# CPJKU/audio_sheet_retrieval

Hardware: AMD Instinct MI355X
Metric: snippet-pairs/sec embedded+ranked (32-d CCA) (higher is better)
Workload: dtype f32

## Files before the change

audio_sheet_retrieval_amd/csrc/conv_wino_kernels.hip:

```cpp
#include <hip/hip_runtime.h>
#include <stdint.h>
#include <stdlib.h>
#include <algorithm>
#include <vector>
#include "asr_kernels.h"
#include "repack_elems.inl"
#include "wino_tile_order.h"

#ifndef ASR_WINOG_ABL
#define ASR_WINOG_ABL 0
#endif

namespace asr {

typedef float floatx4w __attribute__((ext_vector_type(4)));
typedef float float2w __attribute__((ext_vector_type(2)));

#ifndef ASR_WINO_ASMREAD
#define ASR_WINO_ASMREAD 1
#endif
#ifndef ASR_WINO_BUFDMA
#define ASR_WINO_BUFDMA 1
#endif

struct WinoArgs {
    const float *in;
    const float *wpk;
    const float *bnp;
    float *out;
    int N, H, W, OH, OW;
    int RY, RX;
    int MY, MX;
    int nmy, nmx;
    int tiles_y, tiles_x;
    int coutp;
    int C4P, RP;
    int total;
    int per;
    double *stats;
    BnBwdFuse bf;
    const void *raw;
    const float *w1;
    const float *bn1;
};

#ifndef ASR_WINO_PKADD
#define ASR_WINO_PKADD 1
#endif
__device__ __forceinline__ float ssub(float a, float b) {
    float r;
    asm("v_sub_f32 %0, %1, %2" : "=v"(r) : "v"(a), "v"(b));
    return r;
}
__device__ __forceinline__ float2w psub(float2w a, float2w b) {
    if (ASR_WINO_PKADD) return a - b;
    return float2w{ssub(a[0], b[0]), ssub(a[1], b[1])};
}
__device__ __forceinline__ floatx4w psub(floatx4w a, floatx4w b) {
    if (ASR_WINO_PKADD) return a - b;
    return floatx4w{ssub(a[0], b[0]), ssub(a[1], b[1]), ssub(a[2], b[2]), ssub(a[3], b[3])};
}
__device__ __forceinline__ float sadd(float a, float b) {
    float r;
    asm("v_add_f32 %0, %1, %2" : "=v"(r) : "v"(a), "v"(b));
    return r;
}
// ... 7 lines not shown
}

__device__ float4 g_wino_zero[4];

template <int NTV>
__device__ __forceinline__ void wino_stats_store(double *stats, int row, int cout, int col0, int lane,
                                                 const double (&s1)[NTV], const double (&s2)[NTV]) {
    const int g = lane >> 4, n = lane & 15;
#pragma unroll
    for (int nt = 0; nt < NTV; ++nt) {
        double a = s1[nt], b = s2[nt];
        a += __shfl_xor(a, 16); b += __shfl_xor(b, 16);
        a += __shfl_xor(a, 32); b += __shfl_xor(b, 32);
        const int ch = col0 + nt * 16 + n;
        if (g == 0 && ch < cout) {
            stats[((size_t)row * 2) * cout + ch] = a;
            stats[((size_t)row * 2 + 1) * cout + ch] = b;
        }
    }
}

__device__ __forceinline__ float elu_fastw(float y) { return y > 0.0f ? y : __expf(y) - 1.0f; }

template <int CIN, int COUT, bool POOL, int NTW, int KB, int WAVES, int MINW, int RMAX, bool RAW, int PW = 0,
          int IN_MODE = 0>
__global__ __launch_bounds__(64 * (WAVES + PW), MINW) void conv3x3_wino(WinoArgs a) {
    constexpr int KS = CIN / 4;
    constexpr int NB = CIN / 8;
    constexpr bool REM = (CIN % 8) != 0;
    constexpr int NCH = NB / KB;
    constexpr int WROW = NTW * 16;
    constexpr int WS = NTW == 2 ? 48 : WROW;
    constexpr int C4 = CIN / 4;
    constexpr int T = 64 * (WAVES + PW);
    static_assert(NB % KB == 0, "chunking must divide the channel blocks");
    static_assert(PW == 0 || (!RAW && NTW * 16 >= COUT), "producer builds: deterministic path, one n-group");
    extern __shared__ __align__(16) float lds[];
    const int tid = threadIdx.x, lane = tid & 63;
    const int wave = __builtin_amdgcn_readfirstlane(tid >> 6);
    const int LW = a.RX + 2, LH = a.RY + 2;
    constexpr int C4P = (C4 & 1) ? C4 : C4 + 1;
    constexpr int CSf = C4P * 4;
    const int RPf = a.RP * 4;
    const int buf_floats = (LH * RPf + 255) & ~255;
    float *w_lds = lds + 2 * buf_floats;
    const int ng = blockIdx.y;
    const int first = blockIdx.x * a.per;
    const int last = min(first + a.per, a.total);
    if (first >= last) return;

    for (int i = tid; i < 16 * KS * 4 * (WROW / 4); i += T) {
        const int row = i / (WROW / 4), q = i - row * (WROW / 4);
        const int col = ng * WROW + q * 4;
        float4 v = make_float4(0.f, 0.f, 0.f, 0.f);
        if (col < a.coutp) v = *reinterpret_cast<const float4 *>(a.wpk + (size_t)row * a.coutp + col);
        *reinterpret_cast<float4 *>(w_lds + row * WS + q * 4) = v;
    }
    constexpr int RMAXE = PW > 0 ? 1 : RMAX;
    int st_g[RMAXE], st_rc[RMAXE];
    if constexpr (PW == 0) {
#pragma unroll
        for (int k = 0; k < RMAX; ++k) {
            const int f = tid + k * T;
            const int r = f / a.RP;
            const int xs = f - r * a.RP - ((r >> 1) & 1);
            const int px = xs / C4P, c = xs - px * C4P;
            const bool real = r < LH && xs >= 0 && px < LW && c < C4;
#if ASR_WINO_BUFDMA
            st_g[k] = real ? (((r - 1) * a.W + (px - 1)) * CIN + c * 4) * 4 : (int)0x80000000;
#else
            st_g[k] = ((r - 1) * a.W + (px - 1)) * CIN + c * 4;
#endif
            st_rc[k] = real ? (r << 16) | px : -1;
        }
    }
    auto fetch = [&](int region, float *buf) {
        if constexpr (PW == 0) {
        const int tx = region % a.tiles_x;
        const int rest = region / a.tiles_x;
        const int ty = rest % a.tiles_y;
        const int img = rest / a.tiles_y;
        const int Y0 = ty * a.RY, X0 = tx * a.RX;
#if ASR_WINO_BUFDMA
        {
            typedef int int4v __attribute__((ext_vector_type(4)));
            const uint64_t ibase = reinterpret_cast<uint64_t>(a.in + (int64_t)img * a.H * a.W * CIN);
            int4v rsrc;
            rsrc.x = (int)(uint32_t)ibase;
            rsrc.y = (int)(uint32_t)(ibase >> 32);
            rsrc.z = a.H * a.W * CIN * 4;
            rsrc.w = 0x00020000;
            const int roff = (Y0 * a.W + X0) * CIN * 4;
            const unsigned lds0 = (unsigned)(uintptr_t)(__attribute__((address_space(3))) void *)buf;
            const bool xedge = X0 < 1 || X0 + LW - 1 > a.W;
            auto dma = [&](int k, int vo) {
                const unsigned m0v = lds0 + (unsigned)((k * T + wave * 64) * 16);
                asm volatile("s_mov_b32 m0, %2\n\ts_nop 0\n\tbuffer_load_dwordx4 %0, %1, 0 offen lds"
                             ::"v"(vo), "s"(rsrc), "s"(m0v)
                             : "memory", "m0");
            };
            if (!__builtin_amdgcn_readfirstlane((int)xedge)) {
#pragma unroll
                for (int k = 0; k < RMAX; ++k) {
                    if ((k * T + wave * 64) * 4 >= buf_floats) break;
// ... 74 lines not shown
#pragma unroll 1
            for (int cg = 0; cg < C4; ++cg) {
                const float *wg = a.w1 + cg * 36;
                float res[4];
#pragma unroll
                for (int c = 0; c < 4; ++c) {
                    const int co = cg * 4 + c;
                    float acc = 0.0f;
#pragma unroll
                    for (int t = 0; t < 9; ++t) acc = fmaf(v[t], wg[c * 9 + t], acc);
                    res[c] = elu_fastw((acc - a.bn1[co]) * a.bn1[C1P + co] + a.bn1[2 * C1P + co]);
                }
                *reinterpret_cast<float4 *>(dst + cg * 4) = make_float4(res[0], res[1], res[2], res[3]);
            }
        }
        }
    };
    const bool producer = PW > 0 && wave >= WAVES;
    if constexpr (PW > 0) {
        if (IN_MODE == 2)
            for (int i = tid; i < 256; i += T) tab255[i] = (float)i / 255.0f;
        __syncthreads();
        if (producer) produce(first, lds);
    } else {
        fetch(first, lds);
#if ASR_WINO_BUFDMA
        asm volatile("s_waitcnt vmcnt(0)" ::: "memory");
#endif
    }
    __syncthreads();

    const int m = lane & 15, g = lane >> 4, n = lane & 15;
    const int tyy = m / a.MX, txx = m - tyy * a.MX;
    int a_row[4];
#pragma unroll
    for (int i = 0; i < 4; ++i)
        a_row[i] = (2 * tyy + i) * RPf + 2 * txx * CSf + ((tyy + (i >> 1)) & 1) * 4;
    const int a_pair = (g >> 1) * 4 + (g & 1) * 2;
    const int a_rem = NB * 8 + g;
    const float *w_lane = w_lds + g * WS + n;
    auto wq_off = [](int q) { return ((q / (16 * NTW)) * 16 + (q / NTW) % 16) * 4 * WS + (q % NTW) * 16; };
    int ey[4], ex[4], eoff[4];
#pragma unroll
    for (int r = 0; r < 4; ++r) {
        const int me = 4 * g + r;
        ey[r] = me / a.MX;
        ex[r] = me - ey[r] * a.MX;
        eoff[r] = (POOL ? ey[r] * a.OW + ex[r] : 2 * ey[r] * a.W + 2 * ex[r]) * COUT + ng * WROW + n;
    }
    float bmean[NTW], bscale[NTW], bbeta[NTW];
#pragma unroll
    for (int nt = 0; nt < NTW; ++nt) {
        const int ch = ng * WROW + nt * 16 + n;
        const bool ok = !RAW && ch < COUT;
        bmean[nt] = ok ? a.bnp[ch] : 0.f;
        bscale[nt] = ok ? a.bnp[a.coutp + ch] : 1.f;
        bbeta[nt] = ok ? a.bnp[2 * a.coutp + ch] : 0.f;
    }
    float bistd[NTW];
    const bool bnb = ASR_BNB_FUSE_BUILD && RAW && a.stats && a.bf.z != nullptr;
#pragma unroll
    for (int nt = 0; nt < NTW; ++nt) {
        const int ch = ng * WROW + nt * 16 + n;
        bistd[nt] = 0.f;
        if (bnb && ch < COUT) {
            bmean[nt] = a.bf.cst[ch]; bistd[nt] = a.bf.cst[COUT + ch];
            bscale[nt] = a.bf.cst[2 * COUT + ch]; bbeta[nt] = a.bf.cst[3 * COUT + ch];
        }
    }

    double st1[NTW], st2[NTW];
#pragma unroll
    for (int nt = 0; nt < NTW; ++nt) { st1[nt] = 0.0; st2[nt] = 0.0; }
    for (int region = first; region < last; ++region) {
    const float *in_lds = lds + ((region - first) & 1) * buf_floats;
    if (region + 1 < last && !(ASR_WINOG_ABL & 1)) {
        if constexpr (PW > 0) {
            if (producer) produce(region + 1, lds + ((region + 1 - first) & 1) * buf_floats);
        } else {
            fetch(region + 1, lds + ((region + 1 - first) & 1) * buf_floats);
        }
    }
    const int tx = region % a.tiles_x;
    const int rest = region / a.tiles_x;
    const int ty = rest % a.tiles_y;
    const int img = rest / a.tiles_y;
    const int Y0 = ty * a.RY, X0 = tx * a.RX;
    for (int mt = producer ? a.nmy * a.nmx : wave; mt < a.nmy * a.nmx; mt += WAVES) {
        const int mty = mt / a.nmx, mtx = mt - mty * a.nmx;
        const int oy = mty * a.MY * 2, ox = mtx * a.MX * 2;
        if (Y0 + oy >= a.H || X0 + ox >= a.W) continue;
        const float *ap = in_lds + oy * RPf + ox * CSf;
        floatx4w acc[16][NTW];
#pragma unroll
        for (int p = 0; p < 16; ++p)
#pragma unroll
            for (int nt = 0; nt < NTW; ++nt) acc[p][nt] = floatx4w{0.f, 0.f, 0.f, 0.f};

#pragma unroll
        for (int ch = 0; ch < NCH + (REM ? 1 : 0); ++ch) {
            if (ch < NCH) {
                float2w dp[4][4][KB];
#if ASR_WINO_ASMREAD
                if (ASR_WINOG_ABL & 32) {
#pragma unroll
                    for (int i = 0; i < 4; ++i)
#pragma unroll
                        for (int j = 0; j < 4; ++j)
#pragma unroll
                            for (int c = 0; c < KB; ++c) dp[i][j][c] = float2w{(float)i, (float)j};
                } else {
#pragma unroll
                    for (int i = 0; i < 4; ++i) {
                        const unsigned la = (unsigned)(uintptr_t)(const __attribute__((address_space(3))) void *)(ap + a_row[i] + a_pair);
#pragma unroll
                        for (int j = 0; j < 4; ++j)
#pragma unroll
                            for (int c = 0; c < KB; ++c)
                                asm volatile("ds_read_b64 %0, %1 offset:%2"
                                             : "=v"(dp[i][j][c])
                                             : "v"(la), "n"((j * CSf + (ch * KB + c) * 8) * 4));
                    }
#pragma unroll
                    for (int c = 0; c < KB; ++c)
                        asm volatile("s_waitcnt lgkmcnt(0)"
                                     : "+v"(dp[0][0][c]), "+v"(dp[0][1][c]), "+v"(dp[0][2][c]), "+v"(dp[0][3][c]),
                                       "+v"(dp[1][0][c]), "+v"(dp[1][1][c]), "+v"(dp[1][2][c]), "+v"(dp[1][3][c]),
                                       "+v"(dp[2][0][c]), "+v"(dp[2][1][c]), "+v"(dp[2][2][c]), "+v"(dp[2][3][c]),
                                       "+v"(dp[3][0][c]), "+v"(dp[3][1][c]), "+v"(dp[3][2][c]), "+v"(dp[3][3][c]));
                }
#else
#pragma unroll
                for (int i = 0; i < 4; ++i)
#pragma unroll
                    for (int j = 0; j < 4; ++j)
#pragma unroll
                        for (int c = 0; c < KB; ++c)
                            dp[i][j][c] = (ASR_WINOG_ABL & 32) ? float2w{(float)i, (float)j}
                                                               : *reinterpret_cast<const float2w *>(ap + a_row[i] + j * CSf + (ch * KB + c) * 8 + a_pair);
#endif
#pragma unroll
                for (int c = 0; c < KB; ++c) {
#pragma unroll
                    for (int j = 0; j < 4; ++j) {
                        const float2w d0 = dp[0][j][c], d1 = dp[1][j][c], d2 = dp[2][j][c], d3 = dp[3][j][c];
                        dp[0][j][c] = psub(d0, d2); dp[1][j][c] = padd(d1, d2); dp[2][j][c] = psub(d2, d1); dp[3][j][c] = psub(d1, d3);
                    }
#pragma unroll
                    for (int i = 0; i < 4; ++i) {
                        const float2w t0 = dp[i][0][c], t1 = dp[i][1][c], t2 = dp[i][2][c], t3 = dp[i][3][c];
                        dp[i][0][c] = psub(t0, t2); dp[i][1][c] = padd(t1, t2); dp[i][2][c] = psub(t2, t1); dp[i][3][c] = psub(t1, t3);
                    }
                }
                constexpr int WQ = 2 * KB * 16 * NTW, WD = 4 * NTW;
                const float *wk = w_lane + (ch * 2 * KB) * (16 * 4 * WS);
                float wv[WQ + WD];
#pragma unroll
                for (int q = 0; q < WD; ++q) wv[q] = wk[wq_off(q)];
#pragma unroll
                for (int q0 = 0; q0 < WQ; q0 += NTW) {
#pragma unroll
                    for (int q = q0; q < q0 + NTW; ++q)
                        wv[q + WD] = (ASR_WINOG_ABL & 16) ? wv[q] : (q + WD < WQ) ? wk[wq_off(q + WD)] : 0.f;
                    __builtin_amdgcn_sched_barrier(0);
#pragma unroll
                    for (int q = q0; q < q0 + NTW; ++q) {
                        const int p = (q / NTW) % 16, c = q / (16 * NTW), nt = q % NTW;
                        acc[p][nt] = __builtin_amdgcn_mfma_f32_16x16x4f32(dp[p >> 2][p & 3][c >> 1][c & 1], wv[q],
                                                                          acc[p][nt], 0, 0, 0);
                    }
                    __builtin_amdgcn_sched_barrier(0);
                }
            } else {
                float dsg[4][4];
#pragma unroll
                for (int i = 0; i < 4; ++i)
#pragma unroll
                    for (int j = 0; j < 4; ++j) dsg[i][j] = (ASR_WINOG_ABL & 32) ? (float)(i + j) : ap[a_row[i] + j * CSf + a_rem];
#pragma unroll
                for (int j = 0; j < 4; ++j) {
                    const float d0 = dsg[0][j], d1 = dsg[1][j], d2 = dsg[2][j], d3 = dsg[3][j];
                    dsg[0][j] = d0 - d2; dsg[1][j] = d1 + d2; dsg[2][j] = d2 - d1; dsg[3][j] = d1 - d3;
                }
#pragma unroll
                for (int i = 0; i < 4; ++i) {
                    const float t0 = dsg[i][0], t1 = dsg[i][1], t2 = dsg[i][2], t3 = dsg[i][3];
                    dsg[i][0] = t0 - t2; dsg[i][1] = t1 + t2; dsg[i][2] = t2 - t1; dsg[i][3] = t1 - t3;
                }
#pragma unroll
                for (int p = 0; p < 16; ++p)
#pragma unroll
                    for (int nt = 0; nt < NTW; ++nt)
                        acc[p][nt] = __builtin_amdgcn_mfma_f32_16x16x4f32(
                            dsg[p >> 2][p & 3], w_lane[((2 * NB * 16 + p) * 4) * WS + nt * 16], acc[p][nt], 0, 0, 0);
            }
        }

        const int py0 = Y0 + oy, px0 = X0 + ox;
        float *obase = POOL ? a.out + (((int64_t)img * a.OH + (py0 >> 1)) * a.OW + (px0 >> 1)) * COUT
                            : a.out + (((int64_t)img * a.H + py0) * a.W + px0) * COUT;
        const int ly = POOL ? a.OH - (py0 >> 1) : (a.H - py0 + 1) >> 1;
        const int lx = POOL ? a.OW - (px0 >> 1) : (a.W - px0 + 1) >> 1;
#pragma unroll
        for (int nt = 0; nt < NTW; ++nt) {
            if (ng * WROW + nt * 16 + n >= COUT) continue;
            floatx4w s0[4], s1[4];
#pragma unroll
            for (int nu = 0; nu < 4; ++nu) {
                s0[nu] = padd(padd(acc[nu][nt], acc[4 + nu][nt]), acc[8 + nu][nt]);
                s1[nu] = psub(psub(acc[4 + nu][nt], acc[8 + nu][nt]), acc[12 + nu][nt]);
            }
            const floatx4w y00 = padd(padd(s0[0], s0[1]), s0[2]), y01 = psub(psub(s0[1], s0[2]), s0[3]);
            const floatx4w y10 = padd(padd(s1[0], s1[1]), s1[2]), y11 = psub(psub(s1[1], s1[2]), s1[3]);
            const bool full = POOL ? (a.MY <= ly && a.MX <= lx) : (py0 + 2 * a.MY <= a.H && px0 + 2 * a.MX <= a.W);
            if (full && !(ASR_WINOG_ABL & 64)) {
#pragma unroll
                for (int r = 0; r < 4; ++r) {
                    float *o = obase + eoff[r] + nt * 16;
                    if (POOL) {
// ... 51 lines not shown
                    if (x1) o[COUT] = v01;
                    if (y1) o[rstride] = v10;
                    if (y1 && x1) o[rstride + COUT] = v11;
                    if (RAW && a.stats) {
                        if (bnb) {
                            const size_t e = (size_t)(o - a.out);
                            const float *zp = a.bf.z + e;
                            float t1 = 0.f, t2 = 0.f;
                            bnb_acc(v00, zp[0], bnb_mult(a.bf.tie, e), bmean[nt], bscale[nt], bbeta[nt], bistd[nt], t1, t2);
                            if (x1) bnb_acc(v01, zp[COUT], bnb_mult(a.bf.tie, e + COUT), bmean[nt], bscale[nt], bbeta[nt], bistd[nt], t1, t2);
                            if (y1) bnb_acc(v10, zp[rstride], bnb_mult(a.bf.tie, e + rstride), bmean[nt], bscale[nt], bbeta[nt], bistd[nt], t1, t2);
                            if (y1 && x1) bnb_acc(v11, zp[rstride + COUT], bnb_mult(a.bf.tie, e + rstride + COUT), bmean[nt], bscale[nt], bbeta[nt], bistd[nt], t1, t2);
                            st1[nt] += (double)t1; st2[nt] += (double)t2;
                        } else {
                        const float w01 = x1 ? v01 : 0.f, w10 = y1 ? v10 : 0.f, w11 = (y1 && x1) ? v11 : 0.f;
                        st1[nt] += (double)((v00 + w01) + (w10 + w11));
                        st2[nt] += (double)((v00 * v00 + w01 * w01) + (w10 * w10 + w11 * w11));
                        }
                    }
                }
            }
        }
    }
#if ASR_WINO_BUFDMA
    if constexpr (PW == 0) asm volatile("s_waitcnt vmcnt(0)" ::: "memory");
#endif
    __syncthreads();
    }
    if (RAW && a.stats)
        wino_stats_store<NTW>(a.stats, (int)blockIdx.x * WAVES + wave, COUT, ng * WROW, lane, st1, st2);
}

struct WinoGArgs {
    const float *in, *wpk, *bnp;
    float *out;
    int N, H, W, OH, OW;
    int coutp;
    int tiles;
    int total;
    WinoTileOrder ord;
    double *stats;
    BnBwdFuse bf;
};

template <int CIN, int COUT, bool POOL, int NT, int WAVES, int MINW, bool RAW>
__global__ __launch_bounds__(64 * WAVES, MINW) void conv3x3_winog(WinoGArgs a) {
    constexpr int KS = CIN / 4, NB = CIN / 8, WROW = NT * 16, T = 64 * WAVES;
    constexpr int WS = NT == 2 ? 48 : WROW;
    constexpr int WD = 4 * NT;
    constexpr int WQ = 32 * NT;
    constexpr bool REM = (CIN % 8) != 0;
    constexpr bool PIPE = (MINW == 1);
    constexpr bool EARLY = !PIPE && !REM;
// ... 357 lines not shown
        wino_stats_store<NT>(a.stats, (int)blockIdx.x * WAVES + wave, COUT, ng * WROW, lane, gst1, gst2);
}

__global__ void wino_pack_kernel(const float *W, int cin, int cout, int dgrad, float *wpk) {
    const int idx = blockIdx.x * blockDim.x + threadIdx.x;
    if (idx >= wino_pack_count(cin, cout, dgrad)) return;
    wino_pack_elem(idx, W, cin, cout, dgrad, wpk);
}

size_t wino_wpack_floats(int cin, int cout) { return (size_t)16 * cin * ((cout + 15) / 16 * 16); }

hipError_t launch_wino_pack(hipStream_t s, const float *W, int cin, int cout, float *wpk, int dgrad) {
    const int kdim = dgrad ? cout : cin, ndim = dgrad ? cin : cout;
    const int total = kdim * ((ndim + 15) / 16 * 16);
    hipLaunchKernelGGL(wino_pack_kernel, dim3((total + 255) / 256), dim3(256), 0, s, W, cin, cout, dgrad, wpk);
    return hipGetLastError();
}

struct WinoVariant {
    int cin, cout, pool, ntw, kb, waves, minw, rmax, raw;
    void (*kernel)(WinoArgs);
    const char *symbol;
    int pw, in_mode;
};
#define ASR_BOOLSTRW_0 "false"
#define ASR_BOOLSTRW_1 "true"
#define ASR_WINO(CIN, COUT, POOL, NTW, KB, WAVES, MINW, RMAX)                                                     \
    { CIN, COUT, POOL, NTW, KB, WAVES, MINW, RMAX, 0,                                                             \
      conv3x3_wino<CIN, COUT, (POOL != 0), NTW, KB, WAVES, MINW, RMAX, false>,                                    \
      "void asr::conv3x3_wino<" #CIN ", " #COUT ", " ASR_BOOLSTRW_##POOL ", " #NTW ", " #KB ", " #WAVES ", " #MINW \
      ", " #RMAX ", false, 0, 0>(asr::WinoArgs)" }
#define ASR_WINOR(CIN, COUT, NTW, KB, WAVES, MINW, RMAX)                                                          \
    { CIN, COUT, 0, NTW, KB, WAVES, MINW, RMAX, 1,                                                                \
      conv3x3_wino<CIN, COUT, false, NTW, KB, WAVES, MINW, RMAX, true>,                                           \
      "void asr::conv3x3_wino<" #CIN ", " #COUT ", false, " #NTW ", " #KB ", " #WAVES ", " #MINW                  \
      ", " #RMAX ", true, 0, 0>(asr::WinoArgs)" }
#define ASR_WINOF1(CIN, COUT, WAVES, MINW, PW, MODE)                                                              \
    { CIN, COUT, 1, 1, 1, WAVES, MINW, 1, 0,                                                                      \
      conv3x3_wino<CIN, COUT, true, 1, 1, WAVES, MINW, 1, false, PW, MODE>,                                       \
      "void asr::conv3x3_wino<" #CIN ", " #COUT ", true, 1, 1, " #WAVES ", " #MINW ", 1, false, " #PW ", " #MODE  \
      ">(asr::WinoArgs)", PW, MODE }
#define ASR_WINOF(CIN, COUT, WAVES, MINW, PW)                                                                     \
    ASR_WINOF1(CIN, COUT, WAVES, MINW, PW, 0), ASR_WINOF1(CIN, COUT, WAVES, MINW, PW, 1),                         \
        ASR_WINOF1(CIN, COUT, WAVES, MINW, PW, 2)
static const WinoVariant g_wino[] = {
    ASR_WINO(12, 12, 1, 1, 1, 4, 3, 8),
    ASR_WINO(12, 12, 1, 1, 1, 8, 3, 6),
    ASR_WINO(12, 24, 0, 2, 1, 4, 2, 8),
    ASR_WINO(12, 24, 0, 2, 1, 8, 2, 6),
    ASR_WINO(12, 24, 0, 1, 1, 4, 3, 8),
    ASR_WINO(24, 24, 1, 2, 1, 4, 2, 8),
    ASR_WINO(24, 24, 1, 2, 1, 8, 2, 6),
    ASR_WINO(24, 24, 1, 1, 3, 4, 2, 10),
    ASR_WINO(24, 24, 1, 1, 1, 8, 2, 6),
    ASR_WINO(24, 48, 0, 1, 3, 4, 2, 10),
    ASR_WINO(24, 48, 0, 1, 1, 8, 2, 8),
    ASR_WINO(24, 48, 0, 2, 1, 8, 2, 6),
    ASR_WINO(48, 48, 1, 1, 2, 4, 2, 12),
    ASR_WINO(48, 48, 1, 1, 2, 8, 2, 10),
    ASR_WINO(48, 48, 1, 1, 1, 8, 2, 8),
    ASR_WINO(48, 48, 0, 1, 2, 4, 2, 12),
    ASR_WINO(48, 48, 0, 1, 2, 8, 2, 10),
    ASR_WINO(48, 48, 0, 1, 1, 8, 2, 8),
    ASR_WINOR(12, 12, 1, 1, 8, 3, 6),
    ASR_WINOR(12, 24, 2, 1, 8, 2, 6),
    ASR_WINOR(12, 12, 1, 1, 4, 3, 8),
    ASR_WINOR(12, 24, 2, 1, 4, 2, 8),
    ASR_WINOR(12, 24, 1, 1, 4, 3, 8),
    ASR_WINOF(12, 12, 4, 4, 4), ASR_WINOF(12, 12, 4, 3, 2), ASR_WINOF(12, 12, 8, 3, 4), ASR_WINOF(12, 12, 8, 4, 8),
    ASR_WINOF(12, 12, 4, 3, 4),
};
static const int g_num_wino = (int)(sizeof(g_wino) / sizeof(g_wino[0]));

static int wino_lds_layout(int cin, int LW, int MY, int MX, int *c4p_out, int *rp_out) {
    const int c4 = cin / 4;
    const int c4p = (c4 & 1) ? c4 : c4 + 1;
    int best_rp = 0, best = 1 << 30;
    for (int extra = 1; extra <= 8; ++extra) {
        const int rp = LW * c4p + extra;
        int worst = 0;
        for (int half = 0; half < 2; ++half)
            for (int i = 0; i < 4; ++i) {
                int seen[64][32], nseen[64] = {0};
                int cycles = 1;
                for (int l = 0; l < 32; ++l) {
                    const int lane = half * 32 + l;
                    const int m = lane & 15, g = lane >> 4;
                    const int tyy = m / MX, txx = m % MX;
                    const int fl = ((2 * tyy + i) * rp + 2 * txx * c4p + ((tyy + (i >> 1)) & 1)) * 4 + (g >> 1) * 4 + (g & 1) * 2;
                    for (int w = 0; w < 2; ++w) {
                        const int bank = (fl + w) & 63;
                        bool dup = false;
                        for (int q = 0; q < nseen[bank]; ++q) dup = dup || seen[bank][q] == fl + w;
                        if (!dup) seen[bank][nseen[bank]++] = fl + w;
                        cycles = std::max(cycles, nseen[bank]);
                    }
                }
                worst = std::max(worst, cycles);
            }
        if (worst < best) { best = worst; best_rp = rp; }
    }
    *c4p_out = c4p;
    *rp_out = best_rp;
    return best;
}

static void enumerate_wino(int vi, int H, int W, int lds_budget, std::vector<ConvPlan> &out) {
    const WinoVariant &v = g_wino[vi];
    const int nt = (v.cout + 15) / 16;
    const int ngroups = (nt + v.ntw - 1) / v.ntw;
    const int w_bytes = 16 * v.cin * (v.ntw == 2 ? 48 : v.ntw * 16) * 4;
    static const int shapes[4][2] = {{2, 8}, {4, 4}, {8, 2}, {16, 1}};
    const int ty_img = (H + 1) / 2, tx_img = (W + 1) / 2;
    for (const auto &sh : shapes) {
        const int MY = sh[0], MX = sh[1];
        const int max_my = (ty_img + MY - 1) / MY, max_mx = (tx_img + MX - 1) / MX;
        for (int nmy = 1; nmy <= max_my; ++nmy) {
            for (int nmx = 1; nmx <= max_mx; ++nmx) {
                const int RY = nmy * MY * 2, RX = nmx * MX * 2;
                int c4p = 0, rp = 0;
                const int rd_cycles = wino_lds_layout(v.cin, RX + 2, MY, MX, &c4p, &rp);
                const int patch_f4 = (RY + 2) * rp;
                const int lds = 2 * ((patch_f4 * 16 + 1023) & ~1023) + w_bytes + (v.pw ? 1024 : 0);
                if (lds > lds_budget) continue;
                if (!v.pw && patch_f4 > v.rmax * 64 * v.waves) continue;
                const int n_mt = nmy * nmx;
                if (n_mt > 16 * v.waves) continue;
                const int tiles_y = (H + RY - 1) / RY, tiles_x = (W + RX - 1) / RX;
                const double per_wave = (double)((n_mt + v.waves - 1) / v.waves);
                const double mfma = 16.0 * (v.cin / 4) * v.ntw * 32.0;
                const double valu = (16.0 * (v.cin / 4) + 110.0 * v.ntw) * 4.0 + (rd_cycles - 1) * 8.0 * v.cin;
                double stage = (double)v.rmax * 16.0 * 4.0;
                if (v.pw) {
                    const double prod = std::ceil((RY + 2.0) * (RX + 2.0) / (64.0 * v.pw)) * 330.0 * 4.0;
                    const double cons = (16.0 * (v.cin / 4) * v.ntw * 32.0 + (16.0 * (v.cin / 4) + 110.0 * v.ntw) * 4.0) *
                                        (double)((n_mt + v.waves - 1) / v.waves);
                    stage = prod > cons ? prod - cons : 0.0;
                }
                ConvPlan bp{};
                bp.cost = ((mfma + valu) * per_wave + stage + 800.0) * tiles_y * tiles_x * ngroups;
                bp.TH = RY; bp.TW = RX; bp.NI = MY;
                bp.tiles_y = tiles_y; bp.tiles_x = tiles_x;
                bp.lds_bytes = lds;
                bp.tile_floats = nmy * 1000 + nmx;
                bp.c4p = c4p; bp.rp = rp;
                bp.cin = v.cin; bp.cout = v.cout; bp.pool = v.pool;
                bp.H = H; bp.W = W;
                bp.OH = v.pool ? H / 2 : H;
                bp.OW = v.pool ? W / 2 : W;
                bp.threads = 64 * (v.waves + v.pw);
                bp.variant = 3000 + vi;
                bp.symbol = v.symbol;
                bp.fuse1 = v.pw ? 1 : 0;
                out.push_back(bp);
            }
        }
    }
    std::sort(out.begin(), out.end(), [](const ConvPlan &x, const ConvPlan &y) { return x.cost < y.cost; });
}

static void finish_wino(ConvPlan &bp) {
    const WinoVariant &v = g_wino[bp.variant - 3000];
    for (int mode = 0; mode < (v.pw ? 3 : 1); ++mode)
        (void)hipFuncSetAttribute(reinterpret_cast<const void *>(g_wino[bp.variant - 3000 + mode].kernel),
                                  hipFuncAttributeMaxDynamicSharedMemorySize, 160 * 1024);
    int nb = 0;
    if (hipOccupancyMaxActiveBlocksPerMultiprocessor(&nb, reinterpret_cast<const void *>(v.kernel), bp.threads,
// ... 51 lines not shown
        bp.TH = 2; bp.TW = 32; bp.NI = 16;
        bp.tiles_y = pool ? bp.OH : (H + 1) / 2; bp.tiles_x = pool ? bp.OW : (W + 1) / 2;
        bp.threads = 64 * v.waves;
        bp.lds_bytes = lds;
        bp.blocks_per_cu = std::min(nb, 4);
        bp.cost = (double)bp.tiles_y * bp.tiles_x / 16.0 * ((cout + 15) / 16 + v.nt - 1) / v.nt *
                  (16.0 * (cin / 4) * v.nt * 32.0 + 1500.0);
        bp.variant = 3500 + vi;
        bp.symbol = v.symbol;
        out->push_back(bp);
        if (!raw)
            for (int S : {1}) {
                bp.TH = S;
                bp.cost *= 1.01;
                out->push_back(bp);
            }
    }
}

void conv_candidates_wino(int cin, int cout, int pool, int H, int W, int max_count, std::vector<ConvPlan> *out) {
    static const int use = getenv("ASR_CONV_WINO") ? atoi(getenv("ASR_CONV_WINO")) : 1;
    if (!use) return;
    candidates_winog(cin, cout, pool, H, W, out);
    for (int vi = 0; vi < g_num_wino; ++vi) {
        const WinoVariant &v = g_wino[vi];
        if (v.cin != cin || v.cout != cout || v.pool != pool || v.raw || v.pw) continue;
        for (int budget : {52 * 1024, 78 * 1024, 158 * 1024}) {
            std::vector<ConvPlan> c;
            enumerate_wino(vi, H, W, budget, c);
            int taken = 0;
            for (auto &cand : c) {
                bool dup = false;
                for (auto &o : *out)
                    if (o.variant == cand.variant && o.TH == cand.TH && o.TW == cand.TW && o.NI == cand.NI) dup = true;
                if (dup) continue;
                finish_wino(cand);
                out->push_back(cand);
                if (++taken >= max_count) break;
            }
        }
    }
}

void conv_candidates_wino_fused(int cin, int cout, int pool, int H, int W, int max_count, std::vector<ConvPlan> *out) {
    static const int use = getenv("ASR_CONV_WINO") ? atoi(getenv("ASR_CONV_WINO")) : 1;
    if (!use) return;
    for (int vi = 0; vi < g_num_wino; ++vi) {
        const WinoVariant &v = g_wino[vi];
        if (v.cin != cin || v.cout != cout || v.pool != pool || v.raw || !v.pw || v.in_mode != 0) continue;
// ... 91 lines not shown
        const int slots = std::max(1, num_cus * std::max(1, p.blocks_per_cu) / ngroups);
        int grid = std::min((a.total + waves - 1) / waves, slots);
        if (grid >= 8) grid &= ~7;
        a.stats = v.raw ? stats : nullptr;
        a.bf = (bf && a.stats) ? *bf : BnBwdFuse{nullptr, nullptr, nullptr};
        if (a.stats) {
            (void)stats_clean;
            if (stats_rows) *stats_rows = grid * waves;
        }
        hipLaunchKernelGGL(v.kernel, dim3(grid, ngroups), dim3(p.threads), p.lds_bytes, s, a);
        return hipGetLastError();
    }
    const WinoVariant &v0 = g_wino[p.variant - 3000];
    if (v0.pw && (!f1 || f1->rsz || f1->in_mode < 0 || f1->in_mode > 2)) return hipErrorInvalidValue;
    if ((double)p.H * p.W * p.cin * 4.0 >= 2147483648.0) return hipErrorInvalidValue;
    const WinoVariant &v = v0.pw ? g_wino[p.variant - 3000 + f1->in_mode] : v0;
    WinoArgs a;
    a.raw = nullptr; a.w1 = nullptr; a.bn1 = nullptr;
    if (v.pw) { a.raw = f1->raw; a.w1 = f1->w1; a.bn1 = f1->bn1; }
    a.in = in; a.wpk = wpk; a.bnp = bnp; a.out = out;
    a.N = N; a.H = p.H; a.W = p.W; a.OH = p.OH; a.OW = p.OW;
    a.RY = p.TH; a.RX = p.TW;
    a.MY = p.NI; a.MX = 16 / p.NI;
    a.nmy = p.tile_floats / 1000; a.nmx = p.tile_floats % 1000;
    a.tiles_y = p.tiles_y; a.tiles_x = p.tiles_x;
    a.coutp = (p.cout + 15) / 16 * 16;
    a.C4P = p.c4p; a.RP = p.rp;
    a.total = N * p.tiles_y * p.tiles_x;
    if (a.total == 0) return hipSuccess;
    const int nt = a.coutp / 16;
    const int ngroups = (nt + v.ntw - 1) / v.ntw;
    const int slots = std::max(1, num_cus * std::max(1, p.blocks_per_cu) / ngroups);
    a.per = (a.total + slots - 1) / slots;
    const int grid_x = (a.total + a.per - 1) / a.per;
    a.stats = v.raw ? stats : nullptr;
    a.bf = (bf && a.stats) ? *bf : BnBwdFuse{nullptr, nullptr, nullptr};
    if (a.stats) {
        const int rows = grid_x * (p.threads / 64);
        if (stats_rows) *stats_rows = rows;
    }
    hipLaunchKernelGGL(v.kernel, dim3(grid_x, ngroups), dim3(p.threads), p.lds_bytes, s, a);
    return hipGetLastError();
}

int conv_wino_stats_rows_max(int num_cus) { return num_cus * 8 * 8; }

}
// ... 1 lines not shown
```

Baseline: 304,700.

## Add flat work-walk Winograd conv kernels with LDS ring buffer and pipelined remainder reads

Adds a flat Winograd kernel variant where waves walk a single flattened list of valid micro-tiles across regions, instead of striding over per-region tile grids with idle waves and skipped edge tiles. Input patches are prefetched into an N-slot LDS ring sized by a host check so fetches run ahead of the waves. The remainder-channel data and weights are now read through the pipelined asm path. The planner costs these variants from the flattened item count, and they compete by default. In exchange the kernels use more LDS and extra scalar bookkeeping per step, which may lower occupancy.

```diff
diff --git a/audio_sheet_retrieval_amd/csrc/conv_wino_kernels.hip b/audio_sheet_retrieval_amd/csrc/conv_wino_kernels.hip
--- a/audio_sheet_retrieval_amd/csrc/conv_wino_kernels.hip
+++ b/audio_sheet_retrieval_amd/csrc/conv_wino_kernels.hip
@@ -5,6 +5,7 @@
 #include <vector>
 #include "asr_kernels.h"
 #include "repack_elems.inl"
+#include "wino_flat_walk.h"
 #include "wino_tile_order.h"
 
 #ifndef ASR_WINOG_ABL
@@ -18,6 +19,9 @@
 
 #ifndef ASR_WINO_ASMREAD
 #define ASR_WINO_ASMREAD 1
+#endif
+#ifndef ASR_WINO_REMPIPE
+#define ASR_WINO_REMPIPE 1
 #endif
 #ifndef ASR_WINO_BUFDMA
 #define ASR_WINO_BUFDMA 1
@@ -42,6 +46,7 @@
     const void *raw;
     const float *w1;
     const float *bn1;
+    WinoFlatGeom flat;
 };
 
 #ifndef ASR_WINO_PKADD
@@ -95,9 +100,10 @@
 
 __device__ __forceinline__ float elu_fastw(float y) { return y > 0.0f ? y : __expf(y) - 1.0f; }
 
-template <int CIN, int COUT, bool POOL, int NTW, int KB, int WAVES, int MINW, int RMAX, bool RAW, int PW = 0,
-          int IN_MODE = 0>
-__global__ __launch_bounds__(64 * (WAVES + PW), MINW) void conv3x3_wino(WinoArgs a) {
+template <int CIN, int COUT, bool POOL, int NTW, int KB, int WAVES, int MINW, int RMAX, bool RAW, int PW, int IN_MODE,
+          bool FLAT>
+__device__ __forceinline__ void wino_block(const WinoArgs &a) {
+    static_assert(!FLAT || (!RAW && PW == 0 && (WAVES == 4 || WAVES == 8)), "flat walk: deterministic path, no producers");
     constexpr int KS = CIN / 4;
     constexpr int NB = CIN / 8;
     constexpr bool REM = (CIN % 8) != 0;
@@ -116,7 +122,7 @@
     constexpr int CSf = C4P * 4;
     const int RPf = a.RP * 4;
     const int buf_floats = (LH * RPf + 255) & ~255;
-    float *w_lds = lds + 2 * buf_floats;
+    float *w_lds = lds + (FLAT ? a.flat.nbuf : 2) * buf_floats;
     const int ng = blockIdx.y;
     const int first = blockIdx.x * a.per;
     const int last = min(first + a.per, a.total);
@@ -147,12 +153,13 @@
             st_rc[k] = real ? (r << 16) | px : -1;
         }
     }
+    WinoFlatPos cp{}, it{};
     auto fetch = [&](int region, float *buf) {
         if constexpr (PW == 0) {
-        const int tx = region % a.tiles_x;
+        const int tx = FLAT ? __builtin_amdgcn_readfirstlane(cp.tx) : region % a.tiles_x;
         const int rest = region / a.tiles_x;
-        const int ty = rest % a.tiles_y;
-        const int img = rest / a.tiles_y;
+        const int ty = FLAT ? __builtin_amdgcn_readfirstlane(cp.ty) : rest % a.tiles_y;
+        const int img = FLAT ? __builtin_amdgcn_readfirstlane(cp.img) : rest / a.tiles_y;
         const int Y0 = ty * a.RY, X0 = tx * a.RX;
 #if ASR_WINO_BUFDMA
         {
@@ -273,13 +280,13 @@
             for (int i = tid; i < 256; i += T) tab255[i] = (float)i / 255.0f;
         __syncthreads();
         if (producer) produce(first, lds);
-    } else {
+    } else if constexpr (!FLAT) {
         fetch(first, lds);
 #if ASR_WINO_BUFDMA
         asm volatile("s_waitcnt vmcnt(0)" ::: "memory");
 #endif
     }
-    __syncthreads();
+    if constexpr (!FLAT) __syncthreads();
 
     const int m = lane & 15, g = lane >> 4, n = lane & 15;
     const int tyy = m / a.MX, txx = m - tyy * a.MX;
@@ -323,8 +330,31 @@
     double st1[NTW], st2[NTW];
 #pragma unroll
     for (int nt = 0; nt < NTW; ++nt) { st1[nt] = 0.0; st2[nt] = 0.0; }
-    for (int region = first; region < last; ++region) {
-    const float *in_lds = lds + ((region - first) & 1) * buf_floats;
+    constexpr int LOGW = WAVES == 8 ? 3 : 2;
+    int cp_item = 0, items = 0;
+    if constexpr (FLAT) {
+        items = wino_flat_count(a.flat, first, last);
+        wino_flat_start(a.flat, first, first, &cp);
+        wino_flat_start(a.flat, first, first, &it);
+        for (int s = 0; s < wave; ++s) wino_flat_step(a.flat, &it);
+    }
+    const int region_lo = FLAT ? -1 : first, region_hi = FLAT ? (items + WAVES - 1) >> LOGW : last;
+    for (int region = region_lo; region < region_hi; ++region) {
+    const float *in_lds;
+    int img, Y0, X0;
+    bool have = false;
+    if constexpr (FLAT) {
+        while (cp.region < last && (cp_item >> LOGW) <= region + 1) {
+            fetch(cp.region, lds + __builtin_amdgcn_readfirstlane(cp.slot) * buf_floats);
+            cp_item += cp.vy * cp.vx;
+            wino_flat_next_region(a.flat, &cp);
+        }
+        have = region >= 0 && (region << LOGW) + wave < items;
+        in_lds = lds + __builtin_amdgcn_readfirstlane(it.slot) * buf_floats;
+        img = __builtin_amdgcn_readfirstlane(it.img);
+        Y0 = __builtin_amdgcn_readfirstlane(it.ty) * a.RY; X0 = __builtin_amdgcn_readfirstlane(it.tx) * a.RX;
+    } else {
+    in_lds = lds + ((region - first) & 1) * buf_floats;
     if (region + 1 < last && !(ASR_WINOG_ABL & 1)) {
         if constexpr (PW > 0) {
             if (producer) produce(region + 1, lds + ((region + 1 - first) & 1) * buf_floats);
@@ -335,12 +365,15 @@
     const int tx = region % a.tiles_x;
     const int rest = region / a.tiles_x;
     const int ty = rest % a.tiles_y;
-    const int img = rest / a.tiles_y;
-    const int Y0 = ty * a.RY, X0 = tx * a.RX;
-    for (int mt = producer ? a.nmy * a.nmx : wave; mt < a.nmy * a.nmx; mt += WAVES) {
-        const int mty = mt / a.nmx, mtx = mt - mty * a.nmx;
+    img = rest / a.tiles_y;
+    Y0 = ty * a.RY; X0 = tx * a.RX;
+    }
+    const int mt_end = FLAT ? 1 : a.nmy * a.nmx;
+    for (int mt = FLAT ? (have ? 0 : 1) : producer ? mt_end : wave; mt < mt_end; mt += WAVES) {
+        const int mty = FLAT ? __builtin_amdgcn_readfirstlane(it.mty) : mt / a.nmx;
+        const int mtx = FLAT ? __builtin_amdgcn_readfirstlane(it.mtx) : mt - mty * a.nmx;
         const int oy = mty * a.MY * 2, ox = mtx * a.MX * 2;
-        if (Y0 + oy >= a.H || X0 + ox >= a.W) continue;
+        if (!FLAT && (Y0 + oy >= a.H || X0 + ox >= a.W)) continue;
         const float *ap = in_lds + oy * RPf + ox * CSf;
         floatx4w acc[16][NTW];
 #pragma unroll
@@ -348,6 +381,10 @@
 #pragma unroll
             for (int nt = 0; nt < NTW; ++nt) acc[p][nt] = floatx4w{0.f, 0.f, 0.f, 0.f};
 
+        constexpr bool REMPIPE = ASR_WINO_REMPIPE && ASR_WINO_ASMREAD && !(ASR_WINOG_ABL & 48) && REM && NCH == 1 &&
+                                 NTW == 1 && !RAW && PW == 0;
+        float dsr[4][4];
+        float wrem[4 * NTW];
 #pragma unroll
         for (int ch = 0; ch < NCH + (REM ? 1 : 0); ++ch) {
             if (ch < NCH) {
@@ -371,6 +408,15 @@
                                 asm volatile("ds_read_b64 %0, %1 offset:%2"
                                              : "=v"(dp[i][j][c])
                                              : "v"(la), "n"((j * CSf + (ch * KB + c) * 8) * 4));
+                    }
+                    if constexpr (REMPIPE) {
+#pragma unroll
+                        for (int i = 0; i < 4; ++i) {
+                            const unsigned la = (unsigned)(uintptr_t)(const __attribute__((address_space(3))) void *)(ap + a_row[i] + a_rem);
+#pragma unroll
+                            for (int j = 0; j < 4; ++j)
+                                asm volatile("ds_read_b32 %0, %1 offset:%2" : "=v"(dsr[i][j]) : "v"(la), "n"(j * CSf * 4));
+                        }
                     }
 #pragma unroll
                     for (int c = 0; c < KB; ++c)
@@ -379,6 +425,12 @@
                                        "+v"(dp[1][0][c]), "+v"(dp[1][1][c]), "+v"(dp[1][2][c]), "+v"(dp[1][3][c]),
                                        "+v"(dp[2][0][c]), "+v"(dp[2][1][c]), "+v"(dp[2][2][c]), "+v"(dp[2][3][c]),
                                        "+v"(dp[3][0][c]), "+v"(dp[3][1][c]), "+v"(dp[3][2][c]), "+v"(dp[3][3][c]));
+                    if constexpr (REMPIPE)
+                        asm volatile(""
+                                     : "+v"(dsr[0][0]), "+v"(dsr[0][1]), "+v"(dsr[0][2]), "+v"(dsr[0][3]),
+                                       "+v"(dsr[1][0]), "+v"(dsr[1][1]), "+v"(dsr[1][2]), "+v"(dsr[1][3]),
+                                       "+v"(dsr[2][0]), "+v"(dsr[2][1]), "+v"(dsr[2][2]), "+v"(dsr[2][3]),
+                                       "+v"(dsr[3][0]), "+v"(dsr[3][1]), "+v"(dsr[3][2]), "+v"(dsr[3][3]));
                 }
 #else
 #pragma unroll
@@ -412,7 +464,8 @@
                 for (int q0 = 0; q0 < WQ; q0 += NTW) {
 #pragma unroll
                     for (int q = q0; q < q0 + NTW; ++q)
-                        wv[q + WD] = (ASR_WINOG_ABL & 16) ? wv[q] : (q + WD < WQ) ? wk[wq_off(q + WD)] : 0.f;
+                        wv[q + WD] = (ASR_WINOG_ABL & 16) ? wv[q] : (q + WD < WQ) ? wk[wq_off(q + WD)]
+                                     : REMPIPE ? w_lane[((2 * NB * 16 + (q + WD - WQ) / NTW) * 4) * WS + ((q + WD - WQ) % NTW) * 16] : 0.f;
                     __builtin_amdgcn_sched_barrier(0);
 #pragma unroll
                     for (int q = q0; q < q0 + NTW; ++q) {
@@ -422,12 +475,17 @@
                     }
                     __builtin_amdgcn_sched_barrier(0);
                 }
+                if constexpr (REMPIPE) {
+#pragma unroll
+                    for (int r = 0; r < WD; ++r) wrem[r] = wv[WQ + r];
+                }
             } else {
                 float dsg[4][4];
 #pragma unroll
                 for (int i = 0; i < 4; ++i)
 #pragma unroll
-                    for (int j = 0; j < 4; ++j) dsg[i][j] = (ASR_WINOG_ABL & 32) ? (float)(i + j) : ap[a_row[i] + j * CSf + a_rem];
+                    for (int j = 0; j < 4; ++j)
+                        dsg[i][j] = REMPIPE ? dsr[i][j] : (ASR_WINOG_ABL & 32) ? (float)(i + j) : ap[a_row[i] + j * CSf + a_rem];
 #pragma unroll
                 for (int j = 0; j < 4; ++j) {
                     const float d0 = dsg[0][j], d1 = dsg[1][j], d2 = dsg[2][j], d3 = dsg[3][j];
@@ -438,14 +496,35 @@
                     const float t0 = dsg[i][0], t1 = dsg[i][1], t2 = dsg[i][2], t3 = dsg[i][3];
                     dsg[i][0] = t0 - t2; dsg[i][1] = t1 + t2; dsg[i][2] = t2 - t1; dsg[i][3] = t1 - t3;
                 }
+                if constexpr (REMPIPE) {
+                    constexpr int RQ = 16 * NTW, WD = 4 * NTW;
+                    float wr[RQ + WD];
+#pragma unroll
+                    for (int r = 0; r < WD; ++r) wr[r] = wrem[r];
+#pragma unroll
+                    for (int r0 = 0; r0 < RQ; r0 += NTW) {
+#pragma unroll
+                        for (int r = r0; r < r0 + NTW; ++r)
+                            wr[r + WD] = (r + WD < RQ) ? w_lane[((2 * NB * 16 + (r + WD) / NTW) * 4) * WS + ((r + WD) % NTW) * 16] : 0.f;
+                        __builtin_amdgcn_sched_barrier(0);
+#pragma unroll
+                        for (int r = r0; r < r0 + NTW; ++r)
+                            acc[r / NTW][r % NTW] = __builtin_amdgcn_mfma_f32_16x16x4f32(dsg[(r / NTW) >> 2][(r / NTW) & 3], wr[r],
+                                                                                         acc[r / NTW][r % NTW], 0, 0, 0);
+                        __builtin_amdgcn_sched_barrier(0);
+                    }
+                } else {
 #pragma unroll
                 for (int p = 0; p < 16; ++p)
 #pragma unroll
                     for (int nt = 0; nt < NTW; ++nt)
                         acc[p][nt] = __builtin_amdgcn_mfma_f32_16x16x4f32(
                             dsg[p >> 2][p & 3], w_lane[((2 * NB * 16 + p) * 4) * WS + nt * 16], acc[p][nt], 0, 0, 0);
-            }
-        }
+                }
+            }
+        }
+
+        if constexpr (FLAT) asm volatile("s_waitcnt vmcnt(0)" ::: "memory");
 
         const int py0 = Y0 + oy, px0 = X0 + ox;
         float *obase = POOL ? a.out + (((int64_t)img * a.OH + (py0 >> 1)) * a.OW + (px0 >> 1)) * COUT
@@ -543,13 +622,31 @@
             }
         }
     }
+    if constexpr (FLAT) {
+        if (have) {
+            for (int s = 0; s < WAVES; ++s) wino_flat_step(a.flat, &it);
+        } else {
+            asm volatile("s_waitcnt vmcnt(0)" ::: "memory");
+        }
+    }
 #if ASR_WINO_BUFDMA
-    if constexpr (PW == 0) asm volatile("s_waitcnt vmcnt(0)" ::: "memory");
+    if constexpr (PW == 0 && !FLAT) asm volatile("s_waitcnt vmcnt(0)" ::: "memory");
 #endif
     __syncthreads();
     }
     if (RAW && a.stats)
         wino_stats_store<NTW>(a.stats, (int)blockIdx.x * WAVES + wave, COUT, ng * WROW, lane, st1, st2);
+}
+
+template <int CIN, int COUT, bool POOL, int NTW, int KB, int WAVES, int MINW, int RMAX, bool RAW, int PW = 0,
+          int IN_MODE = 0>
+__global__ __launch_bounds__(64 * (WAVES + PW), MINW) void conv3x3_wino(WinoArgs a) {
+    wino_block<CIN, COUT, POOL, NTW, KB, WAVES, MINW, RMAX, RAW, PW, IN_MODE, false>(a);
+}
+
+template <int CIN, int COUT, bool POOL, int NTW, int KB, int WAVES, int MINW, int RMAX>
+__global__ __launch_bounds__(64 * WAVES, MINW) void conv3x3_wino_flat(WinoArgs a) {
+    wino_block<CIN, COUT, POOL, NTW, KB, WAVES, MINW, RMAX, false, 0, 0, true>(a);
 }
 
 struct WinoGArgs {
@@ -953,6 +1050,7 @@
     void (*kernel)(WinoArgs);
     const char *symbol;
     int pw, in_mode;
+    int flat;
 };
 #define ASR_BOOLSTRW_0 "false"
 #define ASR_BOOLSTRW_1 "true"
@@ -974,6 +1072,11 @@
 #define ASR_WINOF(CIN, COUT, WAVES, MINW, PW)                                                                     \
     ASR_WINOF1(CIN, COUT, WAVES, MINW, PW, 0), ASR_WINOF1(CIN, COUT, WAVES, MINW, PW, 1),                         \
         ASR_WINOF1(CIN, COUT, WAVES, MINW, PW, 2)
+#define ASR_WINOFL(CIN, COUT, POOL, NTW, KB, WAVES, MINW, RMAX)                                                   \
+    { CIN, COUT, POOL, NTW, KB, WAVES, MINW, RMAX, 0,                                                             \
+      conv3x3_wino_flat<CIN, COUT, (POOL != 0), NTW, KB, WAVES, MINW, RMAX>,                                      \
+      "void asr::conv3x3_wino_flat<" #CIN ", " #COUT ", " ASR_BOOLSTRW_##POOL ", " #NTW ", " #KB ", " #WAVES      \
+      ", " #MINW ", " #RMAX ">(asr::WinoArgs)", 0, 0, 1 }
 static const WinoVariant g_wino[] = {
     ASR_WINO(12, 12, 1, 1, 1, 4, 3, 8),
     ASR_WINO(12, 12, 1, 1, 1, 8, 3, 6),
@@ -1000,41 +1103,15 @@
     ASR_WINOR(12, 24, 1, 1, 4, 3, 8),
     ASR_WINOF(12, 12, 4, 4, 4), ASR_WINOF(12, 12, 4, 3, 2), ASR_WINOF(12, 12, 8, 3, 4), ASR_WINOF(12, 12, 8, 4, 8),
     ASR_WINOF(12, 12, 4, 3, 4),
+    ASR_WINOFL(12, 12, 1, 1, 1, 4, 3, 8),
+    ASR_WINOFL(12, 12, 1, 1, 1, 8, 3, 6),
+    ASR_WINOFL(12, 24, 0, 2, 1, 4, 2, 8),
+    ASR_WINOFL(12, 24, 0, 2, 1, 8, 2, 6),
+    ASR_WINOFL(12, 24, 0, 1, 1, 4, 3, 8),
+    ASR_WINOFL(24, 24, 1, 1, 3, 4, 2, 10),
+    ASR_WINOFL(24, 24, 1, 1, 1, 8, 2, 6),
 };
 static const int g_num_wino = (int)(sizeof(g_wino) / sizeof(g_wino[0]));
-
-static int wino_lds_layout(int cin, int LW, int MY, int MX, int *c4p_out, int *rp_out) {
-    const int c4 = cin / 4;
-    const int c4p = (c4 & 1) ? c4 : c4 + 1;
-    int best_rp = 0, best = 1 << 30;
-    for (int extra = 1; extra <= 8; ++extra) {
-        const int rp = LW * c4p + extra;
-        int worst = 0;
-        for (int half = 0; half < 2; ++half)
-            for (int i = 0; i < 4; ++i) {
-                int seen[64][32], nseen[64] = {0};
-                int cycles = 1;
-                for (int l = 0; l < 32; ++l) {
-                    const int lane = half * 32 + l;
-                    const int m = lane & 15, g = lane >> 4;
-                    const int tyy = m / MX, txx = m % MX;
-                    const int fl = ((2 * tyy + i) * rp + 2 * txx * c4p + ((tyy + (i >> 1)) & 1)) * 4 + (g >> 1) * 4 + (g & 1) * 2;
-                    for (int w = 0; w < 2; ++w) {
-                        const int bank = (fl + w) & 63;
-                        bool dup = false;
-                        for (int q = 0; q < nseen[bank]; ++q) dup = dup || seen[bank][q] == fl + w;
-                        if (!dup) seen[bank][nseen[bank]++] = fl + w;
-                        cycles = std::max(cycles, nseen[bank]);
-                    }
-                }
-                worst = std::max(worst, cycles);
-            }
-        if (worst < best) { best = worst; best_rp = rp; }
-    }
-    *c4p_out = c4p;
-    *rp_out = best_rp;
-    return best;
-}
 
 static void enumerate_wino(int vi, int H, int W, int lds_budget, std::vector<ConvPlan> &out) {
     const WinoVariant &v = g_wino[vi];
@@ -1052,7 +1129,12 @@
                 int c4p = 0, rp = 0;
                 const int rd_cycles = wino_lds_layout(v.cin, RX + 2, MY, MX, &c4p, &rp);
                 const int patch_f4 = (RY + 2) * rp;
-                const int lds = 2 * ((patch_f4 * 16 + 1023) & ~1023) + w_bytes + (v.pw ? 1024 : 0);
+                int nbuf = 2;
+                if (v.flat) {
+                    nbuf = wino_flat_ring_min(wino_flat_geom_make(H, W, RY, RX, MY, MX, nmy, nmx, 0), v.waves, 24);
+                    if (!nbuf) continue;
+                }
+                const int lds = nbuf * ((patch_f4 * 16 + 1023) & ~1023) + w_bytes + (v.pw ? 1024 : 0);
                 if (lds > lds_budget) continue;
                 if (!v.pw && patch_f4 > v.rmax * 64 * v.waves) continue;
                 const int n_mt = nmy * nmx;
@@ -1070,10 +1152,16 @@
                 }
                 ConvPlan bp{};
                 bp.cost = ((mfma + valu) * per_wave + stage + 800.0) * tiles_y * tiles_x * ngroups;
+                if (v.flat) {
+                    const WinoFlatGeom fg = wino_flat_geom_make(H, W, RY, RX, MY, MX, nmy, nmx, nbuf);
+                    const double rounds = (double)wino_flat_count(fg, 0, tiles_y * tiles_x) / v.waves;
+                    bp.cost = ((mfma + valu + 400.0) * rounds + (stage + 400.0) * tiles_y * tiles_x) * ngroups;
+                }
                 bp.TH = RY; bp.TW = RX; bp.NI = MY;
                 bp.tiles_y = tiles_y; bp.tiles_x = tiles_x;
                 bp.lds_bytes = lds;
                 bp.tile_floats = nmy * 1000 + nmx;
+                if (v.flat) bp.tile_floats += nbuf * 1000000;
                 bp.c4p = c4p; bp.rp = rp;
                 bp.cin = v.cin; bp.cout = v.cout; bp.pool = v.pool;
                 bp.H = H; bp.W = W;
@@ -1171,9 +1259,15 @@
     static const int use = getenv("ASR_CONV_WINO") ? atoi(getenv("ASR_CONV_WINO")) : 1;
     if (!use) return;
     candidates_winog(cin, cout, pool, H, W, out);
+    const char *fenv = getenv("ASR_WINO_FLAT");
+    const int flat_mode = fenv ? atoi(fenv) : 1;
+    bool has_flat = false;
+    for (int vi = 0; vi < g_num_wino; ++vi)
+        has_flat = has_flat || (g_wino[vi].flat && g_wino[vi].cin == cin && g_wino[vi].cout == cout && g_wino[vi].pool == pool);
     for (int vi = 0; vi < g_num_wino; ++vi) {
         const WinoVariant &v = g_wino[vi];
         if (v.cin != cin || v.cout != cout || v.pool != pool || v.raw || v.pw) continue;
+        if (v.flat ? flat_mode == 0 : (flat_mode == 2 && has_flat)) continue;
         for (int budget : {52 * 1024, 78 * 1024, 158 * 1024}) {
             std::vector<ConvPlan> c;
             enumerate_wino(vi, H, W, budget, c);
@@ -1311,7 +1405,9 @@
     a.N = N; a.H = p.H; a.W = p.W; a.OH = p.OH; a.OW = p.OW;
     a.RY = p.TH; a.RX = p.TW;
     a.MY = p.NI; a.MX = 16 / p.NI;
-    a.nmy = p.tile_floats / 1000; a.nmx = p.tile_floats % 1000;
+    a.nmy = p.tile_floats / 1000 % 1000; a.nmx = p.tile_floats % 1000;
+    a.flat = wino_flat_geom_make(p.H, p.W, p.TH, p.TW, a.MY, a.MX, a.nmy, a.nmx, p.tile_floats / 1000000);
+    if (v.flat && (a.flat.nbuf < 3 || a.flat.tiles_y != p.tiles_y || a.flat.tiles_x != p.tiles_x)) return hipErrorInvalidValue;
     a.tiles_y = p.tiles_y; a.tiles_x = p.tiles_x;
     a.coutp = (p.cout + 15) / 16 * 16;
     a.C4P = p.c4p; a.RP = p.rp;
diff --git a/audio_sheet_retrieval_amd/csrc/wino_flat_walk.h b/audio_sheet_retrieval_amd/csrc/wino_flat_walk.h
--- /dev/null
+++ b/audio_sheet_retrieval_amd/csrc/wino_flat_walk.h
@@ -0,0 +1,142 @@
+#pragma once
+
+#if defined(__HIPCC__)
+#define ASR_FLAT_HD __host__ __device__ __forceinline__
+#else
+#define ASR_FLAT_HD inline
+#endif
+
+namespace asr {
+
+struct WinoFlatGeom {
+    int tiles_x, tiles_y;
+    int nmy, nmx;
+    int vy_last, vx_last;
+    int nbuf;
+};
+
+struct WinoFlatPos {
+    int region;
+    int tx, ty, img;
+    int vy, vx;
+    int slot;
+    int mty, mtx;
+};
+
+inline WinoFlatGeom wino_flat_geom_make(int H, int W, int RY, int RX, int MY, int MX, int nmy, int nmx, int nbuf) {
+    WinoFlatGeom g;
+    g.tiles_y = (H + RY - 1) / RY;
+    g.tiles_x = (W + RX - 1) / RX;
+    g.nmy = nmy; g.nmx = nmx;
+    const int rest_y = H - (g.tiles_y - 1) * RY, rest_x = W - (g.tiles_x - 1) * RX;
+    g.vy_last = (rest_y + 2 * MY - 1) / (2 * MY);
+    g.vx_last = (rest_x + 2 * MX - 1) / (2 * MX);
+    g.nbuf = nbuf;
+    return g;
+}
+
+ASR_FLAT_HD void wino_flat_valid(const WinoFlatGeom &g, WinoFlatPos *p) {
+    p->vy = p->ty == g.tiles_y - 1 ? g.vy_last : g.nmy;
+    p->vx = p->tx == g.tiles_x - 1 ? g.vx_last : g.nmx;
+}
+
+ASR_FLAT_HD void wino_flat_start(const WinoFlatGeom &g, int first, int region, WinoFlatPos *p) {
+    p->region = region;
+    p->tx = region % g.tiles_x;
+    const int rest = region / g.tiles_x;
+    p->ty = rest % g.tiles_y;
+    p->img = rest / g.tiles_y;
+    p->slot = (region - first) % g.nbuf;
+    p->mty = 0; p->mtx = 0;
+    wino_flat_valid(g, p);
+}
+
+ASR_FLAT_HD void wino_flat_next_region(const WinoFlatGeom &g, WinoFlatPos *p) {
+    p->region += 1;
+    p->slot = p->slot + 1 == g.nbuf ? 0 : p->slot + 1;
+    p->tx += 1;
+    if (p->tx == g.tiles_x) {
+        p->tx = 0;
+        p->ty += 1;
+        if (p->ty == g.tiles_y) { p->ty = 0; p->img += 1; }
+    }
+    p->mty = 0; p->mtx = 0;
+    wino_flat_valid(g, p);
+}
+
+ASR_FLAT_HD void wino_flat_step(const WinoFlatGeom &g, WinoFlatPos *p) {
+    p->mtx += 1;
+    if (p->mtx < p->vx) return;
+    p->mtx = 0;
+    p->mty += 1;
+    if (p->mty < p->vy) return;
+    wino_flat_next_region(g, p);
+}
+
+ASR_FLAT_HD int wino_flat_count(const WinoFlatGeom &g, int first, int last) {
+    WinoFlatPos p;
+    wino_flat_start(g, first, first, &p);
+    int n = 0;
+    while (p.region < last) {
+        n += p.vy * p.vx;
+        wino_flat_next_region(g, &p);
+    }
+    return n;
+}
+
+inline bool wino_flat_ring_ok(const WinoFlatGeom &g, int waves) {
+    if (g.nbuf < 3) return false;
+    const int per_img = g.tiles_y * g.tiles_x;
+    for (int r0 = 0; r0 < per_img; ++r0) {
+        WinoFlatPos p;
+        wino_flat_start(g, r0, r0, &p);
+        int n = 0;
+        for (int k = 0; k < g.nbuf - 1; ++k) {
+            n += p.vy * p.vx;
+            wino_flat_next_region(g, &p);
+        }
+        if (n < 2 * waves - 1) return false;
+    }
+    return true;
+}
+
+inline int wino_flat_ring_min(WinoFlatGeom g, int waves, int max_nbuf) {
+    for (g.nbuf = 3; g.nbuf <= max_nbuf; ++g.nbuf)
+        if (wino_flat_ring_ok(g, waves)) return g.nbuf;
+    return 0;
+}
+
+inline int wino_lds_layout(int cin, int LW, int MY, int MX, int *c4p_out, int *rp_out) {
+    const int c4 = cin / 4;
+    const int c4p = (c4 & 1) ? c4 : c4 + 1;
+    int best_rp = 0, best = 1 << 30;
+    for (int extra = 1; extra <= 8; ++extra) {
+        const int rp = LW * c4p + extra;
+        int worst = 0;
+        for (int half = 0; half < 2; ++half)
+            for (int i = 0; i < 4; ++i) {
+                int seen[64][32], nseen[64] = {0};
+                int cycles = 1;
+                for (int l = 0; l < 32; ++l) {
+                    const int lane = half * 32 + l;
+                    const int m = lane & 15, g = lane >> 4;
+                    const int tyy = m / MX, txx = m % MX;
+                    const int fl = ((2 * tyy + i) * rp + 2 * txx * c4p + ((tyy + (i >> 1)) & 1)) * 4 + (g >> 1) * 4 + (g & 1) * 2;
+                    for (int w = 0; w < 2; ++w) {
+                        const int bank = (fl + w) & 63;
+                        bool dup = false;
+                        for (int q = 0; q < nseen[bank]; ++q) dup = dup || seen[bank][q] == fl + w;
+                        if (!dup) seen[bank][nseen[bank]++] = fl + w;
+                        cycles = (cycles > nseen[bank] ? cycles : nseen[bank]);
+                    }
+                }
+                worst = (worst > cycles ? worst : cycles);
+            }
+        if (worst < best) { best = worst; best_rp = rp; }
+    }
+    *c4p_out = c4p;
+    *rp_out = best_rp;
+    return best;
+}
+
+}
```

Result: no change. 305,800 (median of 5 runs) (+0.4%).
